# airl-iisc/MRFP

Hardware: AMD Instinct MI355X
Metric: train images/sec (higher is better)
Workload: dtype bf16; 1 GPU; resnet-101 DeepLabV3+ + MRFP+ (HRFP+NP+ on, HRFP re-drawn every step), 768x768, 16 images/GPU, fwd+bwd+SGD, synthetic 19-class, random-init weights; global_batch=16, parallelism=dp1

## Files before the change

### mrfp_amd/csrc/loss.hip

```cpp
#include "loss_common.hpp"

namespace mrfp {

template <typename T>
__global__ __launch_bounds__(kCeThreads) void ce_fwd_kernel(const T* __restrict__ logits, const int64_t* __restrict__ target,
                                                            int64_t npix, int C, int64_t ignore, float* __restrict__ ws) {
    float nll = 0.f, cnt = 0.f;
    for (int64_t p = (int64_t)blockIdx.x * kCeThreads + threadIdx.x; p < npix; p += (int64_t)gridDim.x * kCeThreads) {
        const int64_t tg = target[p];
        if (tg == ignore || tg < 0 || tg >= C) continue;
        const T* l = logits + p * C;
        float m = -INFINITY;
        for (int c = 0; c < C; ++c) m = fmaxf(m, to_f(l[c]));
        float s = 0.f;
        for (int c = 0; c < C; ++c) s += __expf(to_f(l[c]) - m);
        nll += (m + __logf(s)) - to_f(l[tg]);
        cnt += 1.f;
    }
    ce_store_partial(nll, cnt, ws + 2 * blockIdx.x);
}

__global__ void ce_finalize_kernel(const float* ws, int nblk, float* loss) {
    double a, d;
    ce_reduce_partials(ws, nblk, a, d);
    if (threadIdx.x == 0) {
        loss[0] = (float)(a / d);
        loss[1] = (float)d;
    }
}

template <typename T>
__global__ __launch_bounds__(kCeThreads) void ce_bwd_kernel(const T* __restrict__ logits, const int64_t* __restrict__ target,
                                                            const float* __restrict__ loss, const float* __restrict__ gscale,
                                                            T* __restrict__ dlogits, int64_t npix, int C, int64_t ignore) {
    const float k = (gscale ? gscale[0] : 1.f) / loss[1];
    for (int64_t p = (int64_t)blockIdx.x * kCeThreads + threadIdx.x; p < npix; p += (int64_t)gridDim.x * kCeThreads) {
        const int64_t tg = target[p];
        const T* l = logits + p * C;
        T* d = dlogits + p * C;
        if (tg == ignore || tg < 0 || tg >= C) {
            for (int c = 0; c < C; ++c) d[c] = from_f<T>(0.f);
            continue;
        }
        float m = -INFINITY;
        for (int c = 0; c < C; ++c) m = fmaxf(m, to_f(l[c]));
        float s = 0.f;
        for (int c = 0; c < C; ++c) s += __expf(to_f(l[c]) - m);
        const float inv = 1.f / s;
        for (int c = 0; c < C; ++c) {
            const float pr = __expf(to_f(l[c]) - m) * inv;
            d[c] = from_f<T>((pr - (c == tg ? 1.f : 0.f)) * k);
        }
    }
}

template <typename T>
__global__ __launch_bounds__(kCeThreads) void argmax_hist_kernel(const T* __restrict__ logits,
                                                                 const int64_t* __restrict__ target, int64_t npix, int C,
                                                                 unsigned long long* __restrict__ hist,
                                                                 uint8_t* __restrict__ pred) {
    __shared__ unsigned int lh[kMaxClasses * kMaxClasses];
    for (int i = threadIdx.x; i < C * C; i += kCeThreads) lh[i] = 0;
    __syncthreads();
    for (int64_t p = (int64_t)blockIdx.x * kCeThreads + threadIdx.x; p < npix; p += (int64_t)gridDim.x * kCeThreads) {
        const T* l = logits + p * C;
        float m = to_f(l[0]);
        int am = 0;
        for (int c = 1; c < C; ++c) {
            const float v = to_f(l[c]);
            if (v > m) { m = v; am = c; }
        }
        if (pred) pred[p] = (uint8_t)am;
        if (target) {
            const int64_t tg = target[p];
            if (tg >= 0 && tg < C) atomicAdd(&lh[(int)tg * C + am], 1u);
        }
    }
    __syncthreads();
    if (target)
        for (int i = threadIdx.x; i < C * C; i += kCeThreads)
            if (lh[i]) atomicAdd(&hist[i], (unsigned long long)lh[i]);
}

static int ce_blocks(int64_t npix) {
    int64_t b = (npix + kCeThreads - 1) / kCeThreads;
    if (b > 2048) b = 2048;
    if (b < 1) b = 1;
    return (int)b;
}

}

using namespace mrfp;

extern "C" {

int64_t mrfp_ce_nblocks(int64_t npix) { return ce_blocks(npix); }

int mrfp_ce_fwd(const void* logits, const int64_t* target, int dtype, int64_t npix, int64_t C, int64_t ignore_index,
                float* ws, float* loss, void* stream) {
    MRFP_CHECK(logits && target && ws && loss && npix > 0 && C > 0, "ce_fwd: bad arguments");
    hipStream_t st = (hipStream_t)stream;
    const int nb = ce_blocks(npix);
    return by_dtype(dtype, "ce_fwd", [&](auto t) {
        using T = typename decltype(t)::type;
        hipLaunchKernelGGL((ce_fwd_kernel<T>), dim3(nb), dim3(kCeThreads), 0, st, (const T*)logits, target, npix, (int)C, ignore_index, ws);
        MRFP_LAUNCH_CHECK();
        hipLaunchKernelGGL(ce_finalize_kernel, dim3(1), dim3(256), 0, st, ws, nb, loss);
        MRFP_LAUNCH_CHECK();
        return 0;
    });
}

int mrfp_ce_bwd(const void* logits, const int64_t* target, const float* loss, const float* gscale, void* dlogits,
                int dtype, int64_t npix, int64_t C, int64_t ignore_index, void* stream) {
    MRFP_CHECK(logits && target && loss && dlogits && npix > 0 && C > 0, "ce_bwd: bad arguments");
    hipStream_t st = (hipStream_t)stream;
    const int nb = ce_blocks(npix);
    return by_dtype(dtype, "ce_bwd", [&](auto t) {
        using T = typename decltype(t)::type;
        hipLaunchKernelGGL((ce_bwd_kernel<T>), dim3(nb), dim3(kCeThreads), 0, st, (const T*)logits, target, loss, gscale, (T*)dlogits, npix,
                           (int)C, ignore_index);
        MRFP_LAUNCH_CHECK();
        return 0;
    });
}

int mrfp_argmax_hist(const void* logits, const int64_t* target, int dtype, int64_t npix, int64_t C, int64_t* hist,
                     uint8_t* pred, void* stream) {
    MRFP_CHECK(logits && npix > 0 && C > 0 && C <= kMaxClasses, "argmax_hist: bad arguments (C <= %d)", kMaxClasses);
    MRFP_CHECK(!target || hist, "argmax_hist: target given without hist");
    hipStream_t st = (hipStream_t)stream;
    const int nb = ce_blocks(npix);
    return by_dtype(dtype, "argmax_hist", [&](auto t) {
        using T = typename decltype(t)::type;
        hipLaunchKernelGGL((argmax_hist_kernel<T>), dim3(nb), dim3(kCeThreads), 0, st, (const T*)logits, target, npix, (int)C,
                           (unsigned long long*)hist, pred);
        MRFP_LAUNCH_CHECK();
        return 0;
    });
}

}

namespace mrfp {


template <typename T, int CP>
__global__ __launch_bounds__(kCeThreads) void upsample_ce_fwd_kernel(const T* __restrict__ P, int ld, const int64_t* __restrict__ target,
                                                                     int B, int Hi, int Wi, int H, int W, int C, int64_t ignore,
                                                                     float* __restrict__ ws) {
    const int64_t npix = (int64_t)B * H * W;
    float nll = 0.f, cnt = 0.f;
    for (int64_t p = (int64_t)blockIdx.x * kCeThreads + threadIdx.x; p < npix; p += (int64_t)gridDim.x * kCeThreads) {
        const int64_t tg = target[p];
        if (tg == ignore || tg < 0 || tg >= C) continue;
        const int b = (int)(p / ((int64_t)H * W)), rem = (int)(p - (int64_t)b * H * W);
        const int oh = rem / W, ow = rem - oh * W;
        float z[CP];
        up_logits<T, CP>(P, ld, Hi, Wi, H, W, C, b, oh, ow, z);
        float m = -INFINITY;
#pragma unroll
        for (int c = 0; c < CP; ++c) if (c < C) m = fmaxf(m, z[c]);
        float s = 0.f, zt = 0.f;
#pragma unroll
        for (int c = 0; c < CP; ++c)
            if (c < C) { s += __expf(z[c] - m); zt = (c == (int)tg) ? z[c] : zt; }
        nll += (m + __logf(s)) - zt;
        cnt += 1.f;
    }
    ce_store_partial(nll, cnt, ws + 2 * blockIdx.x);
}

template <typename T, int CP>
__global__ __launch_bounds__(kCeThreads) void upsample_ce_bwd_kernel(const T* __restrict__ P, int ld, const int64_t* __restrict__ target,
                                                                     const float* __restrict__ loss, const float* __restrict__ gscale,
                                                                     T* __restrict__ dlogits, int Cd, int B, int Hi, int Wi, int H,
                                                                     int W, int C, int64_t ignore) {
    const int64_t npix = (int64_t)B * H * W;
    const float k = (gscale ? gscale[0] : 1.f) / loss[1];
    for (int64_t p = (int64_t)blockIdx.x * kCeThreads + threadIdx.x; p < npix; p += (int64_t)gridDim.x * kCeThreads) {
        const int64_t tg = target[p];
        T* d = dlogits + p * Cd;
        float g[CP];
#pragma unroll
        for (int c = 0; c < CP; ++c) g[c] = 0.f;
        const bool valid = !(tg == ignore || tg < 0 || tg >= C);
        if (valid) {
            const int b = (int)(p / ((int64_t)H * W)), rem = (int)(p - (int64_t)b * H * W);
            const int oh = rem / W, ow = rem - oh * W;
            up_logits<T, CP>(P, ld, Hi, Wi, H, W, C, b, oh, ow, g);
            float m = -INFINITY;
#pragma unroll
            for (int c = 0; c < CP; ++c) if (c < C) m = fmaxf(m, g[c]);
            float s = 0.f;
#pragma unroll
            for (int c = 0; c < CP; ++c) { g[c] = c < C ? __expf(g[c] - m) : 0.f; s += g[c]; }
            const float inv = 1.f / s;
#pragma unroll
            for (int c = 0; c < CP; ++c) g[c] = c < C ? (g[c] * inv - (c == (int)tg ? 1.f : 0.f)) * k : 0.f;
        }
        store_class_row<T, CP>(d, Cd, g);
    }
}


}

extern "C" {

int mrfp_upsample_ce_fwd(const void* P, int64_t ld, const int64_t* target, int dtype, int64_t B, int64_t Hi, int64_t Wi,
                         int64_t H, int64_t W, int64_t C, int64_t ignore_index, float* ws, float* loss, void* stream) {
    MRFP_CHECK(P && target && ws && loss && B > 0 && Hi > 0 && Wi > 0 && H > 0 && W > 0 && C > 0 && C <= mrfp::kMaxClasses,
               "upsample_ce_fwd: bad arguments");
    if (int rc = mrfp::class_pitch_check("upsample_ce_fwd", P, ld, nullptr, 0, false, dtype, C)) return rc;
    hipStream_t st = (hipStream_t)stream;
    const int nb = mrfp::ce_blocks(B * H * W);
    if (int rc = mrfp::by_dtype_class_pad<mrfp::kMaxClasses>(dtype, "upsample_ce_fwd", (int)C, [&](auto t, auto cp) {
            using T = typename decltype(t)::type;
            hipLaunchKernelGGL((mrfp::upsample_ce_fwd_kernel<T, decltype(cp)::value>), dim3(nb), dim3(mrfp::kCeThreads), 0, st, (const T*)P,
                               (int)ld, target, (int)B, (int)Hi, (int)Wi, (int)H, (int)W, (int)C, ignore_index, ws);
        }))
        return rc;
    hipLaunchKernelGGL(mrfp::ce_finalize_kernel, dim3(1), dim3(256), 0, st, ws, nb, loss);
    MRFP_LAUNCH_CHECK();
    return 0;
}

int mrfp_upsample_ce_bwd(const void* P, int64_t ld, const int64_t* target, const float* loss, const float* gscale,
                         void* dlogits, int64_t Cd, int dtype, int64_t B, int64_t Hi, int64_t Wi, int64_t H, int64_t W,
                         int64_t C, int64_t ignore_index, void* stream) {
    MRFP_CHECK(P && target && loss && dlogits && B > 0 && Hi > 0 && Wi > 0 && H > 0 && W > 0 && C > 0 && C <= mrfp::kMaxClasses,
               "upsample_ce_bwd: bad arguments");
    if (int rc = mrfp::class_pitch_check("upsample_ce_bwd", P, ld, dlogits, Cd, false, dtype, C)) return rc;
    hipStream_t st = (hipStream_t)stream;
    const int nb = mrfp::ce_blocks(B * H * W);
    return mrfp::by_dtype_class_pad<mrfp::kMaxClasses>(dtype, "upsample_ce_bwd", (int)C, [&](auto t, auto cp) {
        using T = typename decltype(t)::type;
        hipLaunchKernelGGL((mrfp::upsample_ce_bwd_kernel<T, decltype(cp)::value>), dim3(nb), dim3(mrfp::kCeThreads), 0, st, (const T*)P,
                           (int)ld, target, loss, gscale, (T*)dlogits, (int)Cd, (int)B, (int)Hi, (int)Wi, (int)H, (int)W, (int)C,
                           ignore_index);
    });
}

}

namespace mrfp {

constexpr int kCeDenseMaxC = 8192;

__device__ __forceinline__ void ce_stage_weights(float* sw, const float* __restrict__ weight, int64_t wstride, int b, int C) {
    const float* w = weight ? weight + (int64_t)b * wstride : nullptr;
    for (int c = threadIdx.x; c < C; c += kCeThreads) sw[c] = w ? w[c] : 1.f;
    __syncthreads();
    if (threadIdx.x < 64) {
        float s = 0.f;
        for (int c = threadIdx.x; c < C; c += 64) s += sw[c];
        s = wave_sum(s);
        if (threadIdx.x == 0) sw[C] = s;
    }
    __syncthreads();
}

__device__ __forceinline__ float ce_w_bwd_factor(const float* __restrict__ loss, const float* __restrict__ gscale, int mode, int b) {
    const float g = gscale ? gscale[0] : 1.f;
    if (mode == MRFP_CE_SUM) return g;
    return g / loss[mode == MRFP_CE_IMAGE_MEAN ? 1 + b : 1];
}

template <typename T>
__global__ __launch_bounds__(kCeThreads) void ce_w_fwd_kernel(const T* __restrict__ logits, const int64_t* __restrict__ target,
                                                              int64_t HW, int C, int64_t ignore, const float* __restrict__ weight,
                                                              int64_t wstride, float eps, float* __restrict__ ws) {
    extern __shared__ float sw[];
    const int b = blockIdx.y;
    ce_stage_weights(sw, weight, wstride, b, C);
    const float om = 1.f - eps, ec = eps / (float)C;
    const T* lb = logits + (int64_t)b * HW * C;
    const int64_t* tb = target + (int64_t)b * HW;
    float num = 0.f, den = 0.f;
    for (int64_t p = (int64_t)blockIdx.x * kCeThreads + threadIdx.x; p < HW; p += (int64_t)gridDim.x * kCeThreads) {
        const int64_t tg = tb[p];
        if (tg == ignore || tg < 0 || tg >= C) continue;
        const T* l = lb + p * C;
        float m = -INFINITY;
        for (int c = 0; c < C; ++c) m = fmaxf(m, to_f(l[c]));
        float s = 0.f;
        for (int c = 0; c < C; ++c) s += __expf(to_f(l[c]) - m);
        const float lse = m + __logf(s), wt = sw[(int)tg];
        float v = om * wt * (lse - to_f(l[tg]));
        if (eps > 0.f) {
            float a = 0.f;
            for (int c = 0; c < C; ++c) a += sw[c] * (lse - to_f(l[c]));
            v += ec * a;
        }
        num += v;
        den += wt;
    }
    ce_w_store_partial(num, den, ws);
}

template <typename T>
__global__ __launch_bounds__(kCeThreads) void ce_w_bwd_kernel(const T* __restrict__ logits, const int64_t* __restrict__ target,
                                                              const float* __restrict__ loss, const float* __restrict__ gscale,
                                                              T* __restrict__ dlogits, int64_t HW, int C, int64_t ignore,
                                                              const float* __restrict__ weight, int64_t wstride, float eps, int mode) {
    extern __shared__ float sw[];
    const int b = blockIdx.y;
    ce_stage_weights(sw, weight, wstride, b, C);
    const float om = 1.f - eps, ec = eps / (float)C, wsum = sw[C];
    const float k = ce_w_bwd_factor(loss, gscale, mode, b);
    const T* lb = logits + (int64_t)b * HW * C;
    T* db = dlogits + (int64_t)b * HW * C;
    const int64_t* tb = target + (int64_t)b * HW;
    for (int64_t p = (int64_t)blockIdx.x * kCeThreads + threadIdx.x; p < HW; p += (int64_t)gridDim.x * kCeThreads) {
        const int64_t tg = tb[p];
        const T* l = lb + p * C;
        T* d = db + p * C;
        if (tg == ignore || tg < 0 || tg >= C) {
            for (int c = 0; c < C; ++c) d[c] = from_f<T>(0.f);
            continue;
        }
        float m = -INFINITY;
        for (int c = 0; c < C; ++c) m = fmaxf(m, to_f(l[c]));
        float s = 0.f;
        for (int c = 0; c < C; ++c) s += __expf(to_f(l[c]) - m);
        const float inv = 1.f / s, wt = om * sw[(int)tg], A = wt + ec * wsum;
        for (int c = 0; c < C; ++c) {
            const float pr = __expf(to_f(l[c]) - m) * inv;
            d[c] = from_f<T>((pr * A - (c == tg ? wt : 0.f) - ec * sw[c]) * k);
        }
    }
}

struct WeightedCe {
    static constexpr int kLdsFloats = kMaxClasses + 1, kMaxClassPad = kMaxClasses;
    static constexpr double kDenBias = 0.0;
    const int64_t* target; int64_t ignore; const float* weight; int64_t wstride; float eps; int mode;

    __device__ __forceinline__ void stage(float* sw, int b, int C) const { ce_stage_weights(sw, weight, wstride, b, C); }
    __device__ __forceinline__ int64_t label(int64_t tg, int) const { return tg; }
    __device__ __forceinline__ bool valid(int64_t tg, int C) const { return !(tg == ignore || tg < 0 || tg >= C); }

    template <int CP>
    __device__ __forceinline__ void add_loss(const float (&z)[CP], int C, int64_t tg, const float* sw, float& num, float& den) const {
        const float om = 1.f - eps, ec = eps / (float)C;
        float m = -INFINITY;
#pragma unroll
        for (int c = 0; c < CP; ++c) if (c < C) m = fmaxf(m, z[c]);
        float s = 0.f, zt = 0.f;
#pragma unroll
        for (int c = 0; c < CP; ++c)
            if (c < C) { s += __expf(z[c] - m); zt = (c == (int)tg) ? z[c] : zt; }
        const float lse = m + __logf(s), wt = sw[(int)tg];
        float v = om * wt * (lse - zt);
        if (eps > 0.f) {
            float a = 0.f;
#pragma unroll
            for (int c = 0; c < CP; ++c) if (c < C) a += sw[c] * (lse - z[c]);
            v += ec * a;
        }
        num += v;
        den += wt;
    }
};

template <typename T, int CP>
__global__ __launch_bounds__(kCeThreads) void upsample_ce_w_bwd_kernel(const T* __restrict__ P, int ld, const int64_t* __restrict__ target,
                                                                       const float* __restrict__ loss, const float* __restrict__ gscale,
                                                                       T* __restrict__ dlogits, int Cd, int Hi, int Wi, int H, int W,
                                                                       int C, int64_t ignore, const float* __restrict__ weight,
                                                                       int64_t wstride, float eps, int mode) {
    __shared__ float sw[kMaxClasses + 1];
    const int b = blockIdx.y;
    ce_stage_weights(sw, weight, wstride, b, C);
    const float om = 1.f - eps, ec = eps / (float)C, wsum = sw[C];
    const float k = ce_w_bwd_factor(loss, gscale, mode, b);
    const int HW = H * W;
    const int64_t* tb = target + (int64_t)b * HW;
    T* db = dlogits + (int64_t)b * HW * Cd;
    for (int p = blockIdx.x * kCeThreads + threadIdx.x; p < HW; p += gridDim.x * kCeThreads) {
        const int64_t tg = tb[p];
        T* d = db + (int64_t)p * Cd;
        float g[CP];
#pragma unroll
        for (int c = 0; c < CP; ++c) g[c] = 0.f;
        if (!(tg == ignore || tg < 0 || tg >= C)) {
            const int oh = p / W, ow = p - oh * W;
            up_logits<T, CP>(P, ld, Hi, Wi, H, W, C, b, oh, ow, g);
            float m = -INFINITY;
#pragma unroll
            for (int c = 0; c < CP; ++c) if (c < C) m = fmaxf(m, g[c]);
            float s = 0.f;
#pragma unroll
            for (int c = 0; c < CP; ++c) { g[c] = c < C ? __expf(g[c] - m) : 0.f; s += g[c]; }
            const float wt = om * sw[(int)tg], A = (wt + ec * wsum) / s;
            if (eps > 0.f) {
#pragma unroll
                for (int c = 0; c < CP; ++c) g[c] = c < C ? (g[c] * A - (c == (int)tg ? wt : 0.f) - ec * sw[c]) * k : 0.f;
            } else {
#pragma unroll
                for (int c = 0; c < CP; ++c) g[c] = c < C ? (g[c] * A - (c == (int)tg ? wt : 0.f)) * k : 0.f;
            }
        }
        store_class_row<T, CP>(d, Cd, g);
    }
}

static int ce_w_check(const char* who, int64_t B, int64_t C, int64_t wstride, float eps, int mode) {
    MRFP_CHECK(B <= 65535, "%s: at most 65535 images (B=%lld)", who, (long long)B);
    if (int rc = wstride_check(who, wstride, C)) return rc;
    MRFP_CHECK(eps >= 0.f && eps < 1.f, "%s: label smoothing must be in [0, 1) (got %g)", who, (double)eps);
    MRFP_CHECK(mode == MRFP_CE_MEAN || mode == MRFP_CE_SUM || mode == MRFP_CE_IMAGE_MEAN, "%s: unknown mode %d", who, mode);
    return 0;
}

struct Focal {
    static constexpr int kLdsFloats = kMaxClasses + 1, kMaxClassPad = kMaxClasses;
    static constexpr double kDenBias = 0.0;
    const int64_t* target; int64_t ignore; const float* weight; int64_t wstride; float gamma; int mode;

    __device__ __forceinline__ void stage(float* sw, int b, int C) const { ce_stage_weights(sw, weight, wstride, b, C); }
    __device__ __forceinline__ int64_t label(int64_t tg, int) const { return tg; }
    __device__ __forceinline__ bool valid(int64_t tg, int C) const { return !(tg == ignore || tg < 0 || tg >= C); }
    __device__ __forceinline__ float bwd_factor(const float* __restrict__ loss, const float* __restrict__ gscale, int b) const {
        return ce_w_bwd_factor(loss, gscale, mode, b);
    }
    __device__ __forceinline__ float qpow(float q) const { return q > 0.f ? __expf(gamma * __logf(q)) : 0.f; }

    template <int CP>
    __device__ __forceinline__ void add_loss(const float (&z)[CP], int C, int64_t tg, const float* sw, float& num, float& den) const {
        float m = -INFINITY;
#pragma unroll
        for (int c = 0; c < CP; ++c) if (c < C) m = fmaxf(m, z[c]);
        float s = 0.f, so = 0.f, zt = 0.f;
#pragma unroll
        for (int c = 0; c < CP; ++c)
            if (c < C) {
                const float e = __expf(z[c] - m);
                s += e;
                so += (c == (int)tg) ? 0.f : e;
                zt = (c == (int)tg) ? z[c] : zt;
            }
        const float lse = m + __logf(s), wt = sw[(int)tg];
        float v = wt * (lse - zt);
        if (gamma != 0.f) v *= qpow(so / s);
        num += v;
        den += wt;
    }

    template <int CP>
    __device__ __forceinline__ void grad(float (&g)[CP], int C, int64_t tg, const float* sw, float k) const {
        float m = -INFINITY, zt = 0.f;
#pragma unroll
        for (int c = 0; c < CP; ++c)
            if (c < C) { m = fmaxf(m, g[c]); zt = (c == (int)tg) ? g[c] : zt; }
        float s = 0.f, so = 0.f, et = 0.f;
#pragma unroll
        for (int c = 0; c < CP; ++c) {
            g[c] = c < C ? __expf(g[c] - m) : 0.f;
            s += g[c];
            so += (c == (int)tg) ? 0.f : g[c];
            et = (c == (int)tg) ? g[c] : et;
        }
        float F = 1.f;
        if (gamma != 0.f) {
            const float q = so / s, qg = qpow(q), nlp = __logf(s) - (zt - m);
            F = q > 0.f ? qg + gamma * (et / s) * (qg / q) * nlp : 0.f;
        }
        const float wt = sw[(int)tg] * F, A = wt / s;
#pragma unroll
        for (int c = 0; c < CP; ++c) g[c] = c < C ? (g[c] * A - (c == (int)tg ? wt : 0.f)) * k : 0.f;
    }
};

static int focal_check(const char* who, int64_t B, int64_t C, int64_t wstride, float gamma, int mode) {
    MRFP_CHECK(C >= 1 && C <= kMaxClasses, "%s: 1 <= C <= %d (C=%lld)", who, kMaxClasses, (long long)C);
    MRFP_CHECK(gamma >= 0.f && gamma <= 3.0e38f, "%s: gamma must be a finite number >= 0 (got %g)", who, (double)gamma);
    return ce_w_check(who, B, C, wstride, 0.f, mode);
}

constexpr int kHistMaxClasses = 1024;

__global__ void label_counts_clear_kernel(unsigned long long* __restrict__ counts, int n) {
    const int i = blockIdx.x * kCeThreads + threadIdx.x;
    if (i < n) counts[i] = 0ull;
}

__global__ __launch_bounds__(kCeThreads) void label_counts_kernel(const int64_t* __restrict__ target, int64_t HW, int C, int pooled,
                                                                  unsigned long long* __restrict__ counts) {
    __shared__ unsigned int lh[kHistMaxClasses];
    for (int i = threadIdx.x; i < C; i += kCeThreads) lh[i] = 0;
    __syncthreads();
    const int64_t* tb = target + (int64_t)blockIdx.y * HW;
    for (int64_t p = (int64_t)blockIdx.x * kCeThreads + threadIdx.x; p < HW; p += (int64_t)gridDim.x * kCeThreads) {
        const int64_t tg = tb[p];
        if (tg >= 0 && tg < C) atomicAdd(&lh[(int)tg], 1u);
    }
    __syncthreads();
    unsigned long long* row = counts + (pooled ? 0 : (int64_t)blockIdx.y * C);
    for (int i = threadIdx.x; i < C; i += kCeThreads)
        if (lh[i]) atomicAdd(&row[i], (unsigned long long)lh[i]);
}

__global__ void label_weights_kernel(const unsigned long long* __restrict__ counts, int rows, int C, double ub, int norm,
                                     float* __restrict__ out) {
    const int i = blockIdx.x * kCeThreads + threadIdx.x;
    if (i >= rows * C) return;
    const unsigned long long* row = counts + (int64_t)(i / C) * C;
    unsigned long long total = 0ull;
    for (int c = 0; c < C; ++c) total += row[c];
    const unsigned long long n = row[i % C];
    double w = 1.0;
    if (n > 0ull) {
        const double f = (double)n / (double)total;
        w = norm ? 1.0 + ub / f : 1.0 + ub * (1.0 - f);
    }
    out[i] = (float)w;
}

}

extern "C" {

int64_t mrfp_ce_w_nblocks(int64_t B, int64_t HW) { return (int64_t)mrfp::ce_w_blocks_x(B, HW) * (B > 0 ? B : 1); }

int64_t mrfp_ce_w_loss_floats(int64_t B, int mode) { return 1 + (mode == MRFP_CE_IMAGE_MEAN ? B : 1); }

int mrfp_ce_w_fwd(const void* logits, const int64_t* target, int dtype, int64_t B, int64_t HW, int64_t C, int64_t ignore_index,
                  const float* weight, int64_t wstride, float smoothing, int mode, float* ws, float* loss, void* stream) {
    MRFP_CHECK(logits && target && ws && loss && B > 0 && HW > 0 && C > 0 && C <= mrfp::kCeDenseMaxC,
               "ce_w_fwd: bad arguments (C <= %d)", mrfp::kCeDenseMaxC);
    if (int rc = mrfp::ce_w_check("ce_w_fwd", B, C, wstride, smoothing, mode)) return rc;
    hipStream_t st = (hipStream_t)stream;
    const int nbx = mrfp::ce_w_blocks_x(B, HW);
    const size_t lds = (size_t)(C + 1) * sizeof(float);
    return mrfp::by_dtype(dtype, "ce_w_fwd", [&](auto t) {
        using T = typename decltype(t)::type;
        hipLaunchKernelGGL((mrfp::ce_w_fwd_kernel<T>), dim3(nbx, (unsigned)B), dim3(mrfp::kCeThreads), lds, st, (const T*)logits, target, HW,
                           (int)C, ignore_index, weight, wstride, smoothing, ws);
        MRFP_LAUNCH_CHECK();
        hipLaunchKernelGGL(mrfp::ce_w_finalize_kernel<mrfp::WeightedCe>, dim3(1), dim3(256), 0, st, ws, nbx, (int)B, mode, loss);
        MRFP_LAUNCH_CHECK();
        return 0;
    });
}

int mrfp_ce_w_bwd(const void* logits, const int64_t* target, const float* loss, const float* gscale, void* dlogits, int dtype,
                  int64_t B, int64_t HW, int64_t C, int64_t ignore_index, const float* weight, int64_t wstride, float smoothing,
                  int mode, void* stream) {
    MRFP_CHECK(logits && target && loss && dlogits && B > 0 && HW > 0 && C > 0 && C <= mrfp::kCeDenseMaxC,
               "ce_w_bwd: bad arguments (C <= %d)", mrfp::kCeDenseMaxC);
    if (int rc = mrfp::ce_w_check("ce_w_bwd", B, C, wstride, smoothing, mode)) return rc;
    hipStream_t st = (hipStream_t)stream;
    const int nbx = mrfp::ce_w_blocks_x(B, HW);
    const size_t lds = (size_t)(C + 1) * sizeof(float);
    return mrfp::by_dtype(dtype, "ce_w_bwd", [&](auto t) {
        using T = typename decltype(t)::type;
        hipLaunchKernelGGL((mrfp::ce_w_bwd_kernel<T>), dim3(nbx, (unsigned)B), dim3(mrfp::kCeThreads), lds, st, (const T*)logits, target, loss,
                           gscale, (T*)dlogits, HW, (int)C, ignore_index, weight, wstride, smoothing, mode);
        MRFP_LAUNCH_CHECK();
        return 0;
    });
}

int mrfp_upsample_ce_w_fwd(const void* P, int64_t ld, const int64_t* target, int dtype, int64_t B, int64_t Hi, int64_t Wi, int64_t H,
                           int64_t W, int64_t C, int64_t ignore_index, const float* weight, int64_t wstride, float smoothing, int mode,
                           float* ws, float* loss, void* stream) {
    const char* who = "upsample_ce_w_fwd";
    MRFP_CHECK(P && target && ws && loss && B > 0, "%s: bad arguments", who);
    MRFP_CHECK(C >= 1 && C <= mrfp::kMaxClasses, "%s: 1 <= C <= %d (C=%lld)", who, mrfp::kMaxClasses, (long long)C);
    if (int rc = mrfp::ce_w_check(who, B, C, wstride, smoothing, mode)) return rc;
    mrfp::BilinearRows src;
    if (int rc = mrfp::bilinear_rows(who, P, ld, nullptr, 0, false, dtype, Hi, Wi, H, W, C, src)) return rc;
    return mrfp::launch_pixel_loss_fwd(who, dtype, B, src, mrfp::WeightedCe{target, ignore_index, weight, wstride, smoothing, mode}, ws, loss,
                                       (hipStream_t)stream);
}

int mrfp_upsample_ce_w_bwd(const void* P, int64_t ld, const int64_t* target, const float* loss, const float* gscale, void* dlogits,
                           int64_t Cd, int dtype, int64_t B, int64_t Hi, int64_t Wi, int64_t H, int64_t W, int64_t C,
                           int64_t ignore_index, const float* weight, int64_t wstride, float smoothing, int mode, void* stream) {
    const char* who = "upsample_ce_w_bwd";
    MRFP_CHECK(P && target && loss && dlogits && B > 0, "%s: bad arguments", who);
    MRFP_CHECK(C >= 1 && C <= mrfp::kMaxClasses, "%s: 1 <= C <= %d (C=%lld)", who, mrfp::kMaxClasses, (long long)C);
    if (int rc = mrfp::ce_w_check(who, B, C, wstride, smoothing, mode)) return rc;
    mrfp::BilinearRows src;
    if (int rc = mrfp::bilinear_rows(who, P, ld, dlogits, Cd, false, dtype, Hi, Wi, H, W, C, src)) return rc;
    hipStream_t st = (hipStream_t)stream;
    const int nbx = mrfp::ce_w_blocks_x(B, src.HW);
    return mrfp::by_dtype_class_pad<mrfp::kMaxClasses>(dtype, who, src.C, [&](auto t, auto cp) {
        using T = typename decltype(t)::type;
        hipLaunchKernelGGL((mrfp::upsample_ce_w_bwd_kernel<T, decltype(cp)::value>), dim3(nbx, (unsigned)B), dim3(mrfp::kCeThreads), 0, st,
                           (const T*)P, src.ld, target, loss, gscale, (T*)dlogits, src.Cd, src.Hi, src.Wi, src.H, src.W, src.C, ignore_index,
                           weight, wstride, smoothing, mode);
    });
}

int mrfp_focal_fwd(const void* logits, const int64_t* target, int dtype, int64_t B, int64_t HW, int64_t C, int64_t ignore_index,
                   const float* weight, int64_t wstride, float gamma, int mode, float* ws, float* loss, void* stream) {
    const char* who = "focal_fwd";
    MRFP_CHECK(logits && target && ws && loss && B > 0 && HW > 0, "%s: bad arguments", who);
    if (int rc = mrfp::focal_check(who, B, C, wstride, gamma, mode)) return rc;
    return mrfp::launch_pixel_loss_fwd(who, dtype, B, mrfp::DenseRows{logits, nullptr, HW, (int)C},
                                       mrfp::Focal{target, ignore_index, weight, wstride, gamma, mode}, ws, loss, (hipStream_t)stream);
}

int mrfp_focal_bwd(const void* logits, const int64_t* target, const float* loss, const float* gscale, void* dlogits, int dtype,
                   int64_t B, int64_t HW, int64_t C, int64_t ignore_index, const float* weight, int64_t wstride, float gamma, int mode,
                   void* stream) {
    const char* who = "focal_bwd";
    MRFP_CHECK(logits && target && loss && dlogits && B > 0 && HW > 0, "%s: bad arguments", who);
    if (int rc = mrfp::focal_check(who, B, C, wstride, gamma, mode)) return rc;
    return mrfp::launch_pixel_loss_bwd(who, dtype, B, mrfp::DenseRows{logits, dlogits, HW, (int)C},
                                       mrfp::Focal{target, ignore_index, weight, wstride, gamma, mode}, loss, gscale, (hipStream_t)stream);
}

int mrfp_upsample_focal_fwd(const void* P, int64_t ld, const int64_t* target, int dtype, int64_t B, int64_t Hi, int64_t Wi, int64_t H,
                            int64_t W, int64_t C, int64_t ignore_index, const float* weight, int64_t wstride, float gamma, int mode,
                            float* ws, float* loss, void* stream) {
    const char* who = "upsample_focal_fwd";
    MRFP_CHECK(P && target && ws && loss && B > 0, "%s: bad arguments", who);
    if (int rc = mrfp::focal_check(who, B, C, wstride, gamma, mode)) return rc;
    mrfp::BilinearRows src;
    if (int rc = mrfp::bilinear_rows(who, P, ld, nullptr, 0, false, dtype, Hi, Wi, H, W, C, src)) return rc;
    return mrfp::launch_pixel_loss_fwd(who, dtype, B, src, mrfp::Focal{target, ignore_index, weight, wstride, gamma, mode}, ws, loss,
                                       (hipStream_t)stream);
}

int mrfp_upsample_focal_bwd(const void* P, int64_t ld, const int64_t* target, const float* loss, const float* gscale, void* dlogits,
                            int64_t Cd, int dtype, int64_t B, int64_t Hi, int64_t Wi, int64_t H, int64_t W, int64_t C,
                            int64_t ignore_index, const float* weight, int64_t wstride, float gamma, int mode, void* stream) {
    const char* who = "upsample_focal_bwd";
    MRFP_CHECK(P && target && loss && dlogits && B > 0, "%s: bad arguments", who);
    if (int rc = mrfp::focal_check(who, B, C, wstride, gamma, mode)) return rc;
    mrfp::BilinearRows src;
    if (int rc = mrfp::bilinear_rows(who, P, ld, dlogits, Cd, false, dtype, Hi, Wi, H, W, C, src)) return rc;
    return mrfp::launch_pixel_loss_bwd(who, dtype, B, src, mrfp::Focal{target, ignore_index, weight, wstride, gamma, mode}, loss, gscale,
                                       (hipStream_t)stream);
}

int mrfp_label_class_weights(const int64_t* target, int64_t B, int64_t HW, int64_t C, double upper_bound, int norm, int batch,
                             int64_t* counts_ws, float* weight_out, void* stream) {
    MRFP_CHECK(target && counts_ws && weight_out && B > 0 && B <= 65535 && HW > 0 && C > 0 && C <= mrfp::kHistMaxClasses,
               "label_class_weights: bad arguments (B <= 65535, C <= %d)", mrfp::kHistMaxClasses);
    hipStream_t st = (hipStream_t)stream;
    const int rows = batch ? 1 : (int)B, n = rows * (int)C;
    unsigned long long* counts = (unsigned long long*)counts_ws;
    hipLaunchKernelGGL(mrfp::label_counts_clear_kernel, dim3((n + mrfp::kCeThreads - 1) / mrfp::kCeThreads), dim3(mrfp::kCeThreads), 0, st,
                       counts, n);
    MRFP_LAUNCH_CHECK();
    hipLaunchKernelGGL(mrfp::label_counts_kernel, dim3(mrfp::ce_w_blocks_x(B, HW), (unsigned)B), dim3(mrfp::kCeThreads), 0, st, target, HW,
                       (int)C, batch ? 1 : 0, counts);
    MRFP_LAUNCH_CHECK();
    hipLaunchKernelGGL(mrfp::label_weights_kernel, dim3((n + mrfp::kCeThreads - 1) / mrfp::kCeThreads), dim3(mrfp::kCeThreads), 0, st,
                       counts, rows, (int)C, upper_bound, norm ? 1 : 0, weight_out);
    MRFP_LAUNCH_CHECK();
    return 0;
}

}
```

Baseline: 307.9 images/sec.

## Tile fused upsample+cross-entropy kernels and stage low-res logits in LDS

Adds a tiled fused bilinear-upsample plus cross-entropy kernel for forward and backward. Each block covers a 64-wide output tile, stages the low-resolution logit patch and its interpolation indices and weights in shared memory, and then computes softmax, NLL or gradients per output pixel. This replaces the per-pixel global gathers of four neighbours. Targets are loaded two at a time when aligned. The new path is on by default via an environment switch and falls back when the LDS footprint exceeds 64KB; it adds diagnostic macros and more template instantiations.

```diff
diff --git a/mrfp_amd/csrc/loss.hip b/mrfp_amd/csrc/loss.hip
--- a/mrfp_amd/csrc/loss.hip
+++ b/mrfp_amd/csrc/loss.hip
@@ -205,6 +205,227 @@
 }
 
 
+#ifndef MRFP_CE_TILE_RPT
+#define MRFP_CE_TILE_RPT 2
+#endif
+#ifndef MRFP_HEAD_DIAG
+#define MRFP_HEAD_DIAG 0
+#endif
+constexpr int kCeTileRpt = MRFP_CE_TILE_RPT;
+constexpr int kCeTileW = 64, kCeTileH = (kCeThreads / 32) * kCeTileRpt;
+constexpr size_t kCeTileMaxLds = 64 * 1024;
+
+template <int CP, typename F>
+__device__ __forceinline__ void for_classes(int C, F&& f) {
+#pragma unroll
+    for (int c = 0; c < CP - 8; ++c) f(c);
+#pragma unroll
+    for (int c = CP - 8; c < CP; ++c) {
+        if (c >= C) break;
+        f(c);
+    }
+}
+
+__device__ __forceinline__ float head_exp(float v) { return MRFP_HEAD_DIAG == 1 ? v : __expf(v); }
+__device__ __forceinline__ float head_log(float v) { return MRFP_HEAD_DIAG == 1 ? v : __logf(v); }
+
+template <typename T, int CP, bool BWD>
+__global__ __launch_bounds__(kCeThreads) void upsample_ce_tile_kernel(const T* __restrict__ P, int ld, const int64_t* __restrict__ target,
+                                                                      const float* __restrict__ loss, const float* __restrict__ gscale,
+                                                                      T* __restrict__ dlogits, int Cd, int Hi, int Wi, int H, int W, int C,
+                                                                      int64_t ignore, float* __restrict__ ws, int tiles_x, int tiles_y,
+                                                                      int per, int rem, int vec_target) {
+    constexpr int EPC = 16 / (int)sizeof(T), NCH = CP / EPC, PS = NCH | 1;
+    using Chunk = VecT<T, EPC>;
+    extern __shared__ __attribute__((aligned(16))) unsigned char ce_tile_lds[];
+    Chunk* img = reinterpret_cast<Chunk*>(ce_tile_lds);
+    __shared__ int s_ri[kCeTileH], s_ci[kCeTileW];
+    __shared__ float s_rl[kCeTileH], s_cl[kCeTileW];
+    __builtin_assume(C > CP - 8);
+    __builtin_assume(C <= CP);
+
+    const int tid = threadIdx.x, lane = tid & 31, trow = tid >> 5;
+    const float sh = up_scale(Hi, H), sw = up_scale(Wi, W);
+    float k = 0.f;
+    if constexpr (BWD) k = (gscale ? gscale[0] : 1.f) / loss[1];
+    float nll = 0.f, cnt = 0.f;
+
+    const int bx = blockIdx.x;
+    const int t0 = bx * per + (bx < rem ? bx : rem), count = per + (bx < rem ? 1 : 0);
+    int tx = t0 % tiles_x, q = t0 / tiles_x;
+    int ty = q % tiles_y, b = q / tiles_y;
+
+    for (int it = 0; it < count; ++it) {
+        const int oh0 = ty * kCeTileH, ow0 = tx * kCeTileW;
+        int64_t tg[kCeTileRpt][2];
+        const int ow = ow0 + 2 * lane;
+#pragma unroll
+        for (int rr = 0; rr < kCeTileRpt; ++rr) {
+            const int oh = oh0 + trow + rr * (kCeThreads / 32);
+            tg[rr][0] = tg[rr][1] = -1;
+            if (oh < H && ow < W) {
+                const int64_t* tp = target + ((size_t)b * H + oh) * W + ow;
+                if (vec_target) {
+                    const VecT<int64_t, 2> v = *reinterpret_cast<const VecT<int64_t, 2>*>(tp);
+                    tg[rr][0] = v.v[0];
+                    tg[rr][1] = v.v[1];
+                } else {
+                    tg[rr][0] = tp[0];
+                    if (ow + 1 < W) tg[rr][1] = tp[1];
+                }
+            }
+        }
+        const int ohl = min(oh0 + kCeTileH - 1, H - 1), owl = min(ow0 + kCeTileW - 1, W - 1);
+        const int hb = (int)(sh * (float)oh0), wb = (int)(sw * (float)ow0);
+        const int hl = (int)(sh * (float)ohl), wl = (int)(sw * (float)owl);
+        const int nr = hl + (hl < Hi - 1 ? 1 : 0) - hb + 1, nc = wl + (wl < Wi - 1 ? 1 : 0) - wb + 1;
+        if (tid < kCeTileH) {
+            const int oh = min(oh0 + tid, H - 1);
+            const float fh = sh * (float)oh;
+            const int h0 = (int)fh, h1 = h0 + (h0 < Hi - 1 ? 1 : 0);
+            s_ri[tid] = (h0 - hb) | ((h1 - hb) << 16);
+            s_rl[tid] = fh - (float)h0;
+        } else if (tid >= 64 && tid < 64 + kCeTileW) {
+            const int j = tid - 64, owc = min(ow0 + j, W - 1);
+            const float fw = sw * (float)owc;
+            const int w0 = (int)fw, w1 = w0 + (w0 < Wi - 1 ? 1 : 0);
+            s_ci[j] = (w0 - wb) | ((w1 - wb) << 16);
+            s_cl[j] = fw - (float)w0;
+        }
+        for (int r = tid >> 6; r < nr; r += kCeThreads / 64)
+            for (int c = tid & 63; c < nc; c += 64) {
+                const T* src = P + (((size_t)b * Hi + hb + r) * Wi + wb + c) * ld;
+                Chunk* dst = img + (r * nc + c) * PS;
+                Chunk v[NCH];
+#pragma unroll
+                for (int ch = 0; ch < NCH; ++ch)
+                    if (ch * EPC < C) v[ch] = load_raw<T, EPC>(src + ch * EPC);
+#pragma unroll
+                for (int ch = 0; ch < NCH; ++ch)
+                    if (ch * EPC < C) dst[ch] = v[ch];
+            }
+        __syncthreads();
+
+#pragma unroll
+        for (int rr = 0; rr < kCeTileRpt; ++rr) {
+            const int r = trow + rr * (kCeThreads / 32), oh = oh0 + r;
+            if (oh >= H) continue;
+            const int ri = s_ri[r];
+            const float lh1 = s_rl[r], lh0 = 1.f - lh1;
+            const int ro0 = (ri & 0xffff) * nc, ro1 = (ri >> 16) * nc;
+#pragma unroll
+            for (int u = 0; u < 2; ++u) {
+                if (ow + u >= W) continue;
+                const int64_t t = tg[rr][u];
+                const bool valid = !(t == ignore || t < 0 || t >= C);
+                if (!BWD && !valid) continue;
+                float g[CP];
+                if constexpr (BWD) {
+#pragma unroll
+                    for (int c = 0; c < CP; ++c) g[c] = 0.f;
+                }
+                if (valid) {
+                    const int ci = s_ci[2 * lane + u];
+                    const float lw1 = s_cl[2 * lane + u], lw0 = 1.f - lw1;
+                    const Chunk* p00 = img + (ro0 + (ci & 0xffff)) * PS;
+                    const Chunk* p01 = img + (ro0 + (ci >> 16)) * PS;
+                    const Chunk* p10 = img + (ro1 + (ci & 0xffff)) * PS;
+                    const Chunk* p11 = img + (ro1 + (ci >> 16)) * PS;
+#if MRFP_HEAD_DIAG == 2
+                    const Chunk only = p00[0];
+#endif
+                    Chunk ra[NCH], rb[NCH], rc[NCH], rd[NCH];
+#pragma unroll
+                    for (int ch = 0; ch < NCH; ++ch) {
+                        if (ch * EPC < C) {
+#if MRFP_HEAD_DIAG == 2
+                            ra[ch] = rb[ch] = rc[ch] = rd[ch] = only;
+#else
+                            ra[ch] = p00[ch];
+                            rb[ch] = p01[ch];
+                            rc[ch] = p10[ch];
+                            rd[ch] = p11[ch];
+#endif
+                        }
+                    }
+                    float m = -INFINITY;
+                    for_classes<CP>(C, [&](int c) {
+                        const int ch = c / EPC, i = c % EPC;
+                        g[c] = lh0 * (lw0 * to_f(ra[ch].v[i]) + lw1 * to_f(rb[ch].v[i])) + lh1 * (lw0 * to_f(rc[ch].v[i]) + lw1 * to_f(rd[ch].v[i]));
+                        m = fmaxf(m, g[c]);
+                    });
+                    if constexpr (BWD) {
+                        float s = 0.f;
+                        for_classes<CP>(C, [&](int c) {
+                            g[c] = head_exp(g[c] - m);
+                            s += g[c];
+                        });
+                        const float inv = 1.f / s;
+#pragma unroll
+                        for (int c = 0; c < CP; ++c) g[c] = c < C ? (g[c] * inv - (c == (int)t ? 1.f : 0.f)) * k : 0.f;
+                    } else {
+                        float s = 0.f, zt = 0.f;
+                        for_classes<CP>(C, [&](int c) {
+                            s += head_exp(g[c] - m);
+                            zt = (c == (int)t) ? g[c] : zt;
+                        });
+                        nll += (m + head_log(s)) - zt;
+                        cnt += 1.f;
+                    }
+                }
+                if constexpr (BWD) store_class_row<T, CP>(dlogits + (((size_t)b * H + oh) * W + ow + u) * Cd, Cd, g);
+            }
+        }
+        if (++tx == tiles_x) {
+            tx = 0;
+            if (++ty == tiles_y) { ty = 0; ++b; }
+        }
+        if (it + 1 < count) __syncthreads();
+    }
+    if constexpr (!BWD) ce_store_partial(nll, cnt, ws + 2 * blockIdx.x);
+}
+
+static float up_scale_host(int64_t in, int64_t out) { return out > 1 ? (float)(in - 1) / (float)(out - 1) : 0.f; }
+
+static int64_t ce_tile_extent(int64_t in, int64_t out, int tile) {
+    const float s = up_scale_host(in, out);
+    int64_t most = 1;
+    for (int64_t o0 = 0; o0 < out; o0 += tile) {
+        const int64_t ol = o0 + tile - 1 < out - 1 ? o0 + tile - 1 : out - 1;
+        const int i0 = (int)(s * (float)o0), il = (int)(s * (float)ol);
+        const int64_t n = il + (il < in - 1 ? 1 : 0) - i0 + 1;
+        if (n > most) most = n;
+    }
+    return most;
+}
+
+struct CeTilePlan {
+    bool ok;
+    int tiles_x, tiles_y, nb, per, rem, vec_target;
+    size_t lds;
+};
+
+static CeTilePlan ce_tile_plan(int dtype, const int64_t* target, int64_t B, int64_t Hi, int64_t Wi, int64_t H, int64_t W, int64_t C) {
+    static const int tiled = env_switch("MRFP_HEAD_TILED", 1);
+    CeTilePlan p{};
+    if (!tiled || !dtype_known(dtype)) return p;
+    const int64_t tx = (W + kCeTileW - 1) / kCeTileW, ty = (H + kCeTileH - 1) / kCeTileH, nt = B * tx * ty;
+    if (nt >= (1LL << 31)) return p;
+    const int epc = 16 / dtype_bytes(dtype);
+    const int64_t cp = (C + 7) / 8 * 8, ps = (cp / epc) | 1;
+    p.lds = (size_t)(ce_tile_extent(Hi, H, kCeTileH) * ce_tile_extent(Wi, W, kCeTileW) * ps * 16);
+    if (p.lds > kCeTileMaxLds) return p;
+    const int64_t cap = ce_blocks(B * H * W);
+    p.nb = (int)(nt < cap ? nt : cap);
+    p.tiles_x = (int)tx;
+    p.tiles_y = (int)ty;
+    p.per = (int)(nt / p.nb);
+    p.rem = (int)(nt % p.nb);
+    p.vec_target = (W % 2 == 0 && aligned16(target)) ? 1 : 0;
+    p.ok = true;
+    return p;
+}
+
 }
 
 extern "C" {
@@ -215,10 +436,16 @@
                "upsample_ce_fwd: bad arguments");
     if (int rc = mrfp::class_pitch_check("upsample_ce_fwd", P, ld, nullptr, 0, false, dtype, C)) return rc;
     hipStream_t st = (hipStream_t)stream;
-    const int nb = mrfp::ce_blocks(B * H * W);
+    const mrfp::CeTilePlan tp = mrfp::ce_tile_plan(dtype, target, B, Hi, Wi, H, W, C);
+    const int nb = tp.ok ? tp.nb : mrfp::ce_blocks(B * H * W);
     if (int rc = mrfp::by_dtype_class_pad<mrfp::kMaxClasses>(dtype, "upsample_ce_fwd", (int)C, [&](auto t, auto cp) {
             using T = typename decltype(t)::type;
-            hipLaunchKernelGGL((mrfp::upsample_ce_fwd_kernel<T, decltype(cp)::value>), dim3(nb), dim3(mrfp::kCeThreads), 0, st, (const T*)P,
+            if (tp.ok)
+                hipLaunchKernelGGL((mrfp::upsample_ce_tile_kernel<T, decltype(cp)::value, false>), dim3(nb), dim3(mrfp::kCeThreads), tp.lds, st,
+                                   (const T*)P, (int)ld, target, (const float*)nullptr, (const float*)nullptr, (T*)nullptr, 0, (int)Hi, (int)Wi,
+                                   (int)H, (int)W, (int)C, ignore_index, ws, tp.tiles_x, tp.tiles_y, tp.per, tp.rem, tp.vec_target);
+            else
+                hipLaunchKernelGGL((mrfp::upsample_ce_fwd_kernel<T, decltype(cp)::value>), dim3(nb), dim3(mrfp::kCeThreads), 0, st, (const T*)P,
                                (int)ld, target, (int)B, (int)Hi, (int)Wi, (int)H, (int)W, (int)C, ignore_index, ws);
         }))
         return rc;
@@ -234,10 +461,16 @@
                "upsample_ce_bwd: bad arguments");
     if (int rc = mrfp::class_pitch_check("upsample_ce_bwd", P, ld, dlogits, Cd, false, dtype, C)) return rc;
     hipStream_t st = (hipStream_t)stream;
-    const int nb = mrfp::ce_blocks(B * H * W);
+    const mrfp::CeTilePlan tp = mrfp::ce_tile_plan(dtype, target, B, Hi, Wi, H, W, C);
+    const int nb = tp.ok ? tp.nb : mrfp::ce_blocks(B * H * W);
     return mrfp::by_dtype_class_pad<mrfp::kMaxClasses>(dtype, "upsample_ce_bwd", (int)C, [&](auto t, auto cp) {
         using T = typename decltype(t)::type;
-        hipLaunchKernelGGL((mrfp::upsample_ce_bwd_kernel<T, decltype(cp)::value>), dim3(nb), dim3(mrfp::kCeThreads), 0, st, (const T*)P,
+        if (tp.ok)
+            hipLaunchKernelGGL((mrfp::upsample_ce_tile_kernel<T, decltype(cp)::value, true>), dim3(nb), dim3(mrfp::kCeThreads), tp.lds, st,
+                               (const T*)P, (int)ld, target, loss, gscale, (T*)dlogits, (int)Cd, (int)Hi, (int)Wi, (int)H, (int)W, (int)C,
+                               ignore_index, (float*)nullptr, tp.tiles_x, tp.tiles_y, tp.per, tp.rem, tp.vec_target);
+        else
+            hipLaunchKernelGGL((mrfp::upsample_ce_bwd_kernel<T, decltype(cp)::value>), dim3(nb), dim3(mrfp::kCeThreads), 0, st, (const T*)P,
                            (int)ld, target, loss, gscale, (T*)dlogits, (int)Cd, (int)B, (int)Hi, (int)Wi, (int)H, (int)W, (int)C,
                            ignore_index);
     });
```

Result: no change. 309.3 images/sec, median of 6 (+0.5%).
